# NikoBiele/RayTraceHeatTransfer.jl

Measured on AMD Instinct MI355X. Metric: Mrays/sec (exchange-factor trace), 101×101 grey κ=1 enclosure, 1/2/4/8 GPUs, higher is better.
Workload: dtype f64; 1 GPU; 101x101 grey kappa=1 sigma_s=0 unit-square enclosure (BASELINE configs[1]); 1e+08 rays per GPU, emitter rows sharded over 1 GPU(s); n_emitters=10605, rays_per_emitter=9429, parallelism=emitter-rows x1 (one process per GPU), devices_visible=1, seed=1

## Files before the change

raytraceheattransfer.jl_amd/csrc/rthx_api.cpp:

```cpp
#define RTHX_HOST_ONLY_TU 1
#include <hip/hip_runtime.h>

#include <algorithm>
#include <chrono>
#include <cmath>
#include <cstdio>
#include <cstdlib>
#include <cstring>
#include <mutex>
#include <string>
#include <thread>
#include <vector>

#include "../../include/rthx.h"
#include "rthx_grid.h"
#include "rthx_kernels.h"

#include "rthx_common.h"
#include "rthx_domain.h"

using rthx::DevBuf;
using rthx::HostBuf;
using rthx::fail;
using rthx::hip_fail;
// ... 438 lines not shown
      off = a16(off + 4 * cmap.size());
      G.off_cinfo = (int32_t)off;
      off = a16(off + sizeof(rthx::MCoarse) * nc);
      G.off_bsolid = (int32_t)off;
      off = a16(off + 4 * nc);
      G.off_beta = (int32_t)off;
      G.blob_bytes = (int32_t)off;
      off = a16(off + 8 * nc);
      if (ncx == 1) {
        G.off_lay = (int32_t)off;
        off = a16(off + sizeof(rthx::LayerRec) * (size_t)(ncy + 2));
      }
      G.inv_x = (double)nx / (xs[nx] - xs[0]);
      G.inv_y = (double)ny / (ys[ny] - ys[0]);
      G.inv_cx = (double)ncx / (cxs[ncx] - cxs[0]);
      G.inv_cy = (double)ncy / (cys[ncy] - cys[0]);
      if (off <= rthx::kMaxCoarseLdsBytes) {
        G.bytes = (int32_t)off;
        std::vector<uint4> blob((size_t)G.blob_bytes / 16);
        char* b = reinterpret_cast<char*>(blob.data());
        std::memset(b, 0, (size_t)G.blob_bytes);
        std::memcpy(b, xs.data(), 8 * xs.size());
        std::memcpy(b + G.off_ys, ys.data(), 8 * ys.size());
        std::memcpy(b + G.off_cxs, cxs.data(), 8 * cxs.size());
        std::memcpy(b + G.off_cys, cys.data(), 8 * cys.size());
        std::memcpy(b + G.off_cmap, cmap.data(), 4 * cmap.size());
        std::memcpy(b + G.off_cinfo, info.data(), sizeof(rthx::MCoarse) * nc);
        std::vector<uint32_t> bsolid(nc);
        std::vector<double> bbeta((size_t)s.n_bins * nc);
        for (size_t bx = 0; bx < nc; ++bx) {
          const int c = cmap[bx];
          bsolid[bx] = csolid[c];
          for (int bn = 0; bn < s.n_bins; ++bn) bbeta[(size_t)bn * nc + bx] = cbeta_all[(size_t)bn * nc + c];
        }
        std::memcpy(b + G.off_bsolid, bsolid.data(), 4 * nc);
        UP(blob.data(), blob.size(), D.ml_blob);
        UP(bbeta.data(), bbeta.size(), D.ml_bbeta);
        d->ml_mixed.assign((size_t)s.n_bins, 0);
        for (int bn = 0; bn < s.n_bins; ++bn)
          for (size_t bx = 0; bx < nc; ++bx) d->ml_mixed[bn] |= bbeta[(size_t)bn * nc + bx] < 0.0 ? 1 : 0;
        D.ml = G;
      }
    }
  }
  if (d->single_convex && d->axis_rect && !env_flag("RTHX_NO_LAT")) {
    std::vector<double> xs, ys;
    for (size_t f = 0; f < nf; ++f) {
      xs.push_back(fpoly[f].x[0]);
      xs.push_back(fpoly[f].x[1]);
      ys.push_back(fpoly[f].y[0]);
      ys.push_back(fpoly[f].y[2]);
    }
    std::sort(xs.begin(), xs.end());
    xs.erase(std::unique(xs.begin(), xs.end()), xs.end());
    std::sort(ys.begin(), ys.end());
    ys.erase(std::unique(ys.begin(), ys.end()), ys.end());
    const int64_t lnx = (int64_t)xs.size() - 1, lny = (int64_t)ys.size() - 1;
    bool ok = lnx >= 1 && lny >= 1 && lnx * lny == (int64_t)nf && lnx <= rthx::kLatMaxDim && lny <= rthx::kLatMaxDim;
    std::vector<int32_t> map(ok ? (size_t)(lnx * lny) : 0, -1);
    bool identity = ok;
    for (size_t f = 0; f < nf && ok; ++f) {
      const auto ix = std::lower_bound(xs.begin(), xs.end(), fpoly[f].x[0]) - xs.begin();
      const auto iy = std::lower_bound(ys.begin(), ys.end(), fpoly[f].y[0]) - ys.begin();
      ok = ix < lnx && iy < lny && xs[ix + 1] == fpoly[f].x[1] && ys[iy + 1] == fpoly[f].y[2] &&
           map[iy * lnx + ix] < 0;
      if (!ok) break;
      map[iy * lnx + ix] = (int32_t)f;
      identity = identity && (int64_t)f == iy * lnx + ix;
      const bool bnd[4] = {iy == 0, ix == lnx - 1, iy == lny - 1, ix == 0};
      for (int w = 0; w < 4 && ok; ++w) ok = bnd[w] || s.fine_surface[4 * f + w] < 0;
    }
    if (ok) {
      rthx::LatticeLayout L{};
      L.nx = (int32_t)lnx;
      L.ny = (int32_t)lny;
      L.identity = identity ? 1 : 0;
      auto a16 = [](size_t b) { return (b + 15) & ~(size_t)15; };
      size_t off = a16(8 * xs.size());
      L.off_ys = (int32_t)off;
      off = a16(off + 8 * ys.size());
      L.bytes = (int32_t)off;
      L.inv_x = (double)lnx / (xs[lnx] - xs[0]);
      L.inv_y = (double)lny / (ys[lny] - ys[0]);
      std::vector<uint4> blob(off / 16);
      char* b = reinterpret_cast<char*>(blob.data());
      std::memset(b, 0, off);
      std::memcpy(b, xs.data(), 8 * xs.size());
      std::memcpy(b + L.off_ys, ys.data(), 8 * ys.size());
      UP(blob.data(), blob.size(), D.lat_blob);
      if (!identity) UP(map.data(), map.size(), D.lat_map);
      D.lat = L;
    }
  }
#undef UP
  {
    int r3 = upload(d, &d->D, 1, &d->d_dom, "domain record");
    if (r3) return bail(r3);
  }
  *out = d;
  return RTHX_OK;
}

RTHX_EXPORT void rthx_domain_destroy(rthx_domain* dom) {
  if (!dom) return;
  (void)hipSetDevice(dom->device);
  (void)hipStreamSynchronize(dom->stream);
  delete dom;
}

RTHX_EXPORT int rthx_result_create(rthx_result** out) {
  if (!out) return fail(RTHX_EINVAL, "null out");
  *out = new (std::nothrow) rthx_result();
  return *out ? RTHX_OK : fail(RTHX_ENOMEM, "host allocation failed");
}

RTHX_EXPORT void rthx_result_destroy(rthx_result* res) { delete res; }

namespace rthx {

int finish_staged(rthx_result* res, const TallyParams& T, int merge, hipStream_t st, hipEvent_t ev_end,
                  int64_t totals[4]) {
  if (T.n_rows > 0) {
    if (merge == kMergeDense) HIP_TRY(launch_compact(T, st), "row_compact_kernel launch");
    if (merge == kMergeParts) HIP_TRY(launch_part_merge(T, st), "part_merge_kernel launch");
    HIP_TRY(launch_scan(T.row_nnz, T.row_tallied, T.n_rows, T.R, res->row_off.as<int64_t>(),
                        res->totals.as<int64_t>(), st),
            "row_scan_kernel launch");
  } else {
    HIP_TRY(hipMemsetAsync(res->row_off.p, 0, 8, st), "hipMemset");
  }
  HIP_TRY(hipMemcpyAsync(totals, res->totals.p, 32, hipMemcpyDeviceToHost, st), "hipMemcpy totals");
  HIP_TRY(hipStreamSynchronize(st), "row scan");
  const size_t nnz = (size_t)std::max<int64_t>(totals[0], 1);
  HIP_TRY(res->cols.reserve(nnz * 4), "hipMalloc cols");
  HIP_TRY(res->cnt.reserve(nnz * 4), "hipMalloc cnt");
  if (T.n_rows > 0)
    HIP_TRY(launch_pack(T.stage_cols, T.stage_cnt, T.row_cap, res->row_off.as<int64_t>(), T.n_rows,
                        res->cols.as<uint32_t>(), res->cnt.as<uint32_t>(), st),
            "csr_pack_kernel launch");
  HIP_TRY(hipEventRecord(ev_end, st), "hipEventRecord");
  HIP_TRY(hipStreamSynchronize(st), "CSR pack");
  return RTHX_OK;
}

}

namespace {

constexpr uint64_t kLookbackWaitTicks = 25'000'000;

uint64_t lookback_wait_ticks() {
  const char* e = rthx::knob("RTHX_LB_WAIT_US");
  if (e && *e) return (uint64_t)std::strtoull(e, nullptr, 10) * 100;
  return kLookbackWaitTicks;
}

using rthx::TracePlan;
static_assert(rthx::kTallyU16 == 1, "TracePlan::tally default");

constexpr int64_t kMaxHashCap = 16384;

int plan_trace(const rthx_domain* dom, const rthx_trace_args* a, TracePlan& p, int64_t slots = 0) {
  if (a->bin < 0 || a->bin >= dom->n_bins) return fail(RTHX_EINVAL, "bin out of range");
  if (a->rays_per_emitter < 0 || a->rays_per_emitter > 0xFFFFFFFFll)
    return fail(RTHX_ERANGE, "rays_per_emitter must be in [0, 2^32)");
  if (a->emitter_stride < 1 || a->emitter_begin < 0) return fail(RTHX_EINVAL, "bad emitter range");
// ... 836 lines not shown
```

raytraceheattransfer.jl_amd/csrc/rthx_device.h:

```cpp
#pragma once

#include <hip/hip_runtime.h>
#include <stdint.h>

#if defined(__HIP_DEVICE_COMPILE__) && !defined(RTHX_HOST_ONLY_TU)
#define RTHX_GLOBAL __attribute__((address_space(1)))
#else
#define RTHX_GLOBAL
#endif

#ifndef RTHX_PHILOX_OPAQUE_KEY
#define RTHX_PHILOX_OPAQUE_KEY 1
#endif

namespace rthx {

struct DevGrid {
  double ox, oy;
  double inv_x, inv_y;
  int32_t nx, ny;
  int32_t cell_base;
  int32_t reserved;
};

// ... 542 lines not shown
template <bool FAITHFUL>
__device__ __forceinline__ void iso_dir(uint32_t w_th, uint32_t w_ph, const double* cos_tab, double& dx, double& dy) {
  const double u = u32(w_th);
  double st, ct, cphi;
  if (FAITHFUL) {
    const double theta = acos(2.0 * u - 1.0);
    st = sin(theta);
    ct = cos(theta);
    cphi = cos(RTHX_TWO_PI * u32(w_ph));
  } else {
    ct = 2.0 * u - 1.0;
    st = 2.0 * sqrt_unit(__dmul_rn(u, 1.0 - u));
    cphi = cos_2pi_u32(w_ph, cos_tab);
  }
  dx = __dmul_rn(st, cphi);
  dy = ct;
}

template <bool FAITHFUL>
__device__ __forceinline__ void redirect_dir(bool wall, double tx, double ty, uint32_t w1, uint32_t w2,
                                             const double* cos_tab, double& dx, double& dy) {
  if (FAITHFUL) {
    if (wall)
      lambert_dir<true>(tx, ty, w1, w2, cos_tab, dx, dy);
    else
      iso_dir<true>(w1, w2, cos_tab, dx, dy);
    return;
  }
  const double u = u32(w1);
  const float ct_w = (float)sqrt_unit((double)(float)u);
  const double ct = wall ? (double)ct_w : 2.0 * u - 1.0;
  const double arg = wall ? 1.0 - (double)__fmul_rn(ct_w, ct_w) : 4.0 * __dmul_rn(u, 1.0 - u);
  const double st = sqrt_unit(arg);
  const double cpsi = cos_2pi_u32(wall ? f32_draw_word(w2) : w2, cos_tab);
  const double fx = wall ? tx : 1.0, fy = wall ? ty : 0.0;
  const double xl = __dmul_rn(st, cpsi);
  dx = __dmul_rn(fx, xl) + __dmul_rn(-fy, ct);
  dy = __dmul_rn(fy, xl) + __dmul_rn(fx, ct);
}

constexpr int kEmitAny = 0, kEmitVolRect = 2;
template <int EK> struct EmitKind { static constexpr int value = EK; };

template <bool FAITHFUL, int EK = kEmitAny>
__device__ __forceinline__ void emit_volume(const Emitter& e, double eta, const RayWords& rw, const double* cos_tab,
                                            double& px, double& py, double& dx, double& dy) {
  const double R1 = u32(rw.a[0]), R2 = u32(rw.a[1]);
  if (!FAITHFUL && (EK == kEmitVolRect || e.rect)) {
    px = __builtin_fma((double)rw.a[0], e.sx, e.v[0]);
    py = __builtin_fma((double)rw.a[1], e.sy, e.v[1]);
  } else {
    double s1 = FAITHFUL ? sqrt(R1) : sqrt_unit(R1);
    double wa = 1.0 - s1, wb = __dmul_rn(s1, 1.0 - R2), wc = __dmul_rn(s1, R2);
    double Ax = e.v[0], Ay = e.v[1], Bx = e.v[2], By = e.v[3], Cx = e.v[4], Cy = e.v[5];
    if (EK == kEmitVolRect || e.nv == 4) {
      double sel = u32(rw.sw);
      if (!(sel < e.tri_frac)) {
        Ax = e.v[4]; Ay = e.v[5]; Bx = e.v[6]; By = e.v[7]; Cx = e.v[0]; Cy = e.v[1];
      }
    }
    px = __dmul_rn(wa, Ax) + __dmul_rn(wb, Bx) + __dmul_rn(wc, Cx);
    py = __dmul_rn(wa, Ay) + __dmul_rn(wb, By) + __dmul_rn(wc, Cy);
  }
  px = px + __dmul_rn(e.mx - px, eta);
  py = py + __dmul_rn(e.my - py, eta);
  double st, ct, cphi;
  if (FAITHFUL) {
    double u4 = u32(rw.a[2]);
    double theta = acos(1.0 - 2.0 * u4);
    st = sin(theta);
    ct = cos(theta);
    cphi = cos(RTHX_TWO_PI * u32(rw.a[3]));
  } else {
    const double w4 = (double)rw.a[2];
    ct = __builtin_fma(w4, -0x1.0p-31, 1.0);
    const double om = __builtin_fma(w4, -0x1.0p-32, 1.0) * 0x1.0p-32;
    st = 2.0 * sqrt_unit(w4 * om);
    cphi = cos_2pi_u32(rw.a[3], cos_tab);
  }
  dx = __dmul_rn(st, cphi);
  dy = ct;
}

struct SingleCoarse {
  DevPoly poly;
  DevGrid grid;
  uint32_t solid;
  int32_t count;
};

constexpr int kRayContinue = -3;

template <bool UNIFORM, bool SINGLE, bool AXIS>
__device__ __forceinline__ int segment(const DevDomain& D, const TraceParams& P, const SingleCoarse& sc, int& c,
                                       double& px, double& py, double dx, double dy, double& S, double& acc) {
  const double eta = P.eta;
  int k, first, count;
  double u;
  uint32_t solid;
  if (SINGLE) {
    first = 0;
    count = sc.count;
    u = dist_to_cell<AXIS>(px, py, dx, dy, sc.poly, k);
    solid = sc.solid;
  } else {
    first = D.f_offset[c];
    count = D.f_offset[c + 1] - first;
    u = dist_to_cell<AXIS>(px, py, dx, dy, D.c_poly[c], k);
    solid = D.c_solid[c];
  }
  bool gas;
  double beta = 0.0, tau_b = 0.0;
  if (UNIFORM) {
    gas = S < u;
  } else {
    int f0 = SINGLE ? locate_fine(D, sc.grid, first, count, px, py) : locate_fine(D, D.f_grid[c], first, count, px, py);
    if (f0 < 0) return -1;
    beta = D.beta[(size_t)P.bin * D.n_fine + first + f0];
    tau_b = __dmul_rn(beta, u);
    gas = acc + tau_b >= S;
  }
  bool wall = !gas && ((solid >> k) & 1u);
  if (gas || wall) {
    double t = gas ? (UNIFORM ? S : (S - acc) / beta) - eta : u - eta;
    px = px + __dmul_rn(t, dx);
    py = py + __dmul_rn(t, dy);
    int f = SINGLE ? locate_fine(D, sc.grid, first, count, px, py) : locate_fine(D, D.f_grid[c], first, count, px, py);
    if (f < 0) return -1;
    int fg = first + f;
    if (gas) return D.n_surfaces + fg;
    int w;
    dist_to_cell<AXIS>(px, py, dx, dy, D.f_poly[fg], w);
    return D.f_surf[4 * fg + w];
  }
  if (SINGLE) return -1;
  double t = u + eta;
  px = px + __dmul_rn(t, dx);
  py = py + __dmul_rn(t, dy);
  if (UNIFORM) S -= u; else acc += tau_b;
  c = locate_coarse(D, px, py);
  return c < 0 ? -1 : kRayContinue;
}

#ifndef RTHX_LDS
#define RTHX_LDS __attribute__((address_space(3)))
#endif

__device__ __forceinline__ int lattice_index(const double RTHX_LDS* b, int n, double inv, double x) {
  int i;
  __asm__("v_cvt_i32_f64 %0, %1" : "=v"(i) : "v"(__dmul_rn(x - b[0], inv)));
  __asm__("v_med3_i32 %0, %1, 0, %2" : "=v"(i) : "v"(i), "s"(__builtin_amdgcn_readfirstlane(n - 1)));
  const double lo = b[i], hi = b[i + 1];
  if ((lo <= x) & (x < hi)) return i;
  while (i > 0 && x < b[i]) --i;
  while (i < n - 1 && !(x < b[i + 1])) ++i;
  return (b[i] <= x && x < b[i + 1]) ? i : -1;
}

static_assert(kLatMaxDim <= (1 << 12), "j nx + i must fit the 24-bit multiply and its 32-bit byte offsets");
__device__ __forceinline__ int lat_cell(int i, int j, int nx) {
  return (int)(__umul24((uint32_t)j, (uint32_t)nx) + (uint32_t)i);
}

template <class T>
__device__ __forceinline__ T ld_off32(const T RTHX_GLOBAL* base, uint32_t byte_off) {
  return *(const T RTHX_GLOBAL*)((const char RTHX_GLOBAL*)base + byte_off);
}

struct LatticeLds {
  const double RTHX_LDS* xs;
  const double RTHX_LDS* ys;
};

__device__ __forceinline__ LatticeLds lattice_lds_view(const char RTHX_LDS* base, const LatticeLayout& L) {
  LatticeLds v;
  v.xs = (const double RTHX_LDS*)base;
  v.ys = (const double RTHX_LDS*)(base + L.off_ys);
  return v;
}

template <bool UNIFORM, bool INSIDE = false, bool FOUR = false>
__device__ __forceinline__ int segment_lat(const DevDomain& D, const TraceParams& P, const SingleCoarse& sc,
                                           const LatticeLds& L, const LatticeLayout& G, double& px, double& py,
                                           double dx, double dy, double& S, double& acc) {
  const double eta = P.eta;
  int k;
  const double cx0 = sc.poly.x[0], cx1 = sc.poly.x[1], cy0 = sc.poly.y[0], cy1 = sc.poly.y[2];
  double u;
  if (!FOUR && (INSIDE || (cx0 <= px && px < cx1 && cy0 <= py && py < cy1)))
    u = dist_in_box(px, py, dx, dy, dx < 0.0 ? cx0 : cx1, dy < 0.0 ? cy0 : cy1, k);
  else
    u = dist_to_box(px, py, dx, dy, cx0, cx1, cy0, cy1, k);
  bool gas;
  double beta = 0.0, tau_b = 0.0;
  if (UNIFORM) {
    gas = S < u;
  } else {
    const int i0 = lattice_index(L.xs, G.nx, G.inv_x, px), j0 = lattice_index(L.ys, G.ny, G.inv_y, py);
    if (i0 < 0 || j0 < 0) return -1;
    const int f0 = G.identity ? lat_cell(i0, j0, G.nx) : D.lat_map[lat_cell(i0, j0, G.nx)];
    beta = D.beta[(size_t)P.bin * D.n_fine + f0];
    tau_b = __dmul_rn(beta, u);
    gas = acc + tau_b >= S;
  }
  const bool wall = !gas && ((sc.solid >> k) & 1u);
  if (!(gas || wall)) return -1;
  const double t = gas ? (UNIFORM ? S : (S - acc) / beta) - eta : u - eta;
  px = px + __dmul_rn(t, dx);
  py = py + __dmul_rn(t, dy);
  const int i = lattice_index(L.xs, G.nx, G.inv_x, px), j = lattice_index(L.ys, G.ny, G.inv_y, py);
  if (i < 0 || j < 0) return -1;
  const int cell = lat_cell(i, j, G.nx);
  if (gas) return D.n_surfaces + (G.identity ? cell : D.lat_map[cell]);
  const int w = box_hit_in(px, py, dx, dy, dx < 0.0 ? L.xs[i] : L.xs[i + 1], dy < 0.0 ? L.ys[j] : L.ys[j + 1]).wall;
  return ld_off32(D.f_surf, ((uint32_t)(G.identity ? cell : D.lat_map[cell]) << 4) + ((uint32_t)w << 2));
}

#ifndef RTHX_LDS
#define RTHX_LDS __attribute__((address_space(3)))
#endif

template <class T>
__device__ __forceinline__ T ld(const T RTHX_LDS* p) { return *(const T*)p; }
template <class T>
__device__ __forceinline__ T ld(const T RTHX_GLOBAL* p) { return *p; }

struct CoarseLds {
  const DevPoly RTHX_LDS* poly;
  const DevGrid RTHX_LDS* fgrid;
  const double RTHX_LDS* bbox;
  const int32_t RTHX_LDS* first;
  const uint32_t RTHX_LDS* solid;
  const DevCell RTHX_LDS* cells;
  const double RTHX_LDS* beta;
};

__device__ __forceinline__ CoarseLds coarse_lds_view(const char RTHX_LDS* base, const CoarseLayout& L) {
  CoarseLds v;
  v.poly = (const DevPoly RTHX_LDS*)base;
  v.fgrid = (const DevGrid RTHX_LDS*)(base + L.off_fgrid);
  v.bbox = (const double RTHX_LDS*)(base + L.off_bbox);
  v.first = (const int32_t RTHX_LDS*)(base + L.off_first);
  v.solid = (const uint32_t RTHX_LDS*)(base + L.off_solid);
  v.cells = (const DevCell RTHX_LDS*)(base + L.off_cells);
  v.beta = (const double RTHX_LDS*)(base + L.off_beta);
  return v;
}

constexpr int kRayEndGas = -4;
constexpr int kRayEndWall = -5;

template <bool UNIFORM, bool AXIS>
__device__ __forceinline__ int walk_cl(const DevDomain& D, const TraceParams& P, const CoarseLds& L, int& c,
                                       double& px, double& py, double dx, double dy, double& S, double& acc) {
  const double eta = P.eta;
  int k;
  const double u = dist_to_cell<AXIS>(px, py, dx, dy, L.poly[c], k);
  const uint32_t solid = L.solid[c];
  bool gas;
  double beta = 0.0, tau_b = 0.0;
  if (UNIFORM) {
    gas = S < u;
  } else {
    beta = L.beta[c];
    if (beta < 0.0) {
      const int first = L.first[c];
      const DevGrid fg = ld(L.fgrid + c);
      const int f0 = locate_fine(D, fg, first, L.first[c + 1] - first, px, py);
      if (f0 < 0) return -1;
      beta = D.beta[(size_t)P.bin * D.n_fine + first + f0];
    }
    tau_b = __dmul_rn(beta, u);
    gas = acc + tau_b >= S;
  }
  const bool wall = !gas && ((solid >> k) & 1u);
  if (gas || wall) {
    const double t = gas ? (UNIFORM ? S : (S - acc) / beta) - eta : u - eta;
    px = px + __dmul_rn(t, dx);
    py = py + __dmul_rn(t, dy);
    return gas ? kRayEndGas : kRayEndWall;
  }
  const double t = u + eta;
  px = px + __dmul_rn(t, dx);
  py = py + __dmul_rn(t, dy);
  if (UNIFORM) S -= u; else acc += tau_b;
  c = locate(D.c_grid, D, L.cells, L.poly, L.bbox, 0, D.n_coarse, px, py);
  return c < 0 ? -1 : kRayContinue;
}

template <bool AXIS>
__device__ __forceinline__ int end_cl(const DevDomain& D, const CoarseLds& L, int c, double px, double py, double dx,
                                      double dy, bool gas) {
  const int first = L.first[c];
  const DevGrid fg = ld(L.fgrid + c);
  const int f = locate_fine(D, fg, first, L.first[c + 1] - first, px, py);
  if (f < 0) return -1;
  const int fg_idx = first + f;
  if (gas) return D.n_surfaces + fg_idx;
// ... 267 lines not shown
        if (beta < 0.0) {
          const MCoarse m = ld(L.cinfo + L.cmap[cj]);
          int i, j;
          const int f0 = ml_fine(L, G, m, px, py, i, j);
          lost = f0 < 0;
          beta = lost ? 0.0 : D.beta[(size_t)P.bin * D.n_fine + f0];
        }
      }
      accn = acc + __dmul_rn(beta, u);
      gas = accn >= S;
    }
    const bool wall = !gas & ((rec.solid & ybit) != 0u);
    if ((it >= kMaxWalkSteps) | !fast | lost | gas | wall) {
      status = it >= kMaxWalkSteps ? -1 : !fast ? kRaySlowSeg : lost ? -1 : gas ? kRayEndGas : kRayEndWall;
      break;
    }
    const double t = u + eta;
    px = px + __dmul_rn(t, r.dx);
    py = py + __dmul_rn(t, r.dy);
    if (UNIFORM) S -= u; else acc = accn;
    cj += sy;
    ++it;
    if ((uint32_t)__popcll(__ballot(1)) <= stop) break;
  }
  u_end = u;
  B.ci = 0;
  B.cj = cj;
  B.b = cj;
  return status;
}

__device__ __forceinline__ bool relocate_layers(const MLatLds& L, const MLatLayout& G, MBox& B, double px,
                                                double py) {
  const int li = lattice_index(L.cxs, 1, G.inv_cx, px), lj = lattice_index(L.cys, G.ncy, G.inv_cy, py);
  if ((li < 0) | (lj < 0)) return false;
  B.ci = 0;
  B.cj = lj;
  B.b = lj;
  return true;
}

template <bool UNIFORM>
__device__ __forceinline__ void end_move_ml(const DevDomain& D, const TraceParams& P, const MLatLds& L,
                                            const MLatLayout& G, const MBox& B, double& px, double& py,
                                            const MRay& r, double S, double acc, double u_end, bool gas) {
  double t = u_end;
  if (gas) {
    if (UNIFORM) {
      t = S;
    } else {
      double beta = L.beta[B.b];
      if (P.mixed && beta < 0.0) {
        const MCoarse m = ld(L.cinfo + L.cmap[B.b]);
        int i, j;
        beta = D.beta[(size_t)P.bin * D.n_fine + ml_fine(L, G, m, px, py, i, j)];
      }
      t = (S - acc) / beta;
    }
  }
  t = t - P.eta;
  px = px + __dmul_rn(t, r.dx);
  py = py + __dmul_rn(t, r.dy);
}

__device__ __forceinline__ int end_ml(const DevDomain& D, const MLatLds& L, const MLatLayout& G, const MBox& B,
                                      double px, double py, double dx, double dy, bool gas) {
  const MCoarse m = ld(L.cinfo + L.cmap[B.b]);
  int i, j;
  const int fg = ml_fine(L, G, m, px, py, i, j);
  if (fg < 0) return -1;
  if (gas) return D.n_surfaces + fg;
  const int w = box_hit_in(px, py, dx, dy, dx < 0.0 ? L.xs[i] : L.xs[i + 1], dy < 0.0 ? L.ys[j] : L.ys[j + 1]).wall;
  return D.f_surf[4 * fg + w];
}

template <bool UNIFORM, bool FAITHFUL>
__device__ __forceinline__ double free_path(const TraceParams& P, const double* tabs, double u) {
  if (UNIFORM)
    return FAITHFUL ? (P.beta_uniform > 0 ? -log(u) / P.beta_uniform : __builtin_inf())
                    : neg_log_tab(u, tabs + kLogTableOffset) * tabs[kTabInvBeta];
  return FAITHFUL ? -log(u) : neg_log_tab(u, tabs + kLogTableOffset);
}

template <bool UNIFORM, bool FAITHFUL>
__device__ __forceinline__ double free_path_u32(const TraceParams& P, const double* tabs, uint32_t w) {
  if (FAITHFUL) return free_path<UNIFORM, true>(P, tabs, u32(w));
  const double l = neg_log_u32(w, tabs + kLogTableOffset);
  if (UNIFORM) return l * tabs[kTabInvBeta];
  return l;
}

template <int EK = kEmitAny>
__device__ __forceinline__ bool emitter_surface(const Emitter& e) { return EK == kEmitAny ? e.surface : false; }

template <int EK = kEmitAny>
__device__ __forceinline__ RayWords ray_words(const TraceParams& P, const Emitter& e, uint32_t g, uint32_t r,
                                              bool have_pw, uint32_t pw, bool faithful) {
  RayWords rw;
  philox_words(r, g, 0u, (uint32_t)P.bin, P.key0, P.key1, rw.a);
  rw.pw = 0u;
  rw.sw = 0u;
  if (!emitter_surface<EK>(e)) {
    if (have_pw) {
      rw.pw = pw;
    } else {
      uint32_t b[4];
      philox_words(r >> 2, g, 1u, (uint32_t)P.bin, P.key0, P.key1, b);
      const uint32_t j = r & 3u;
      rw.pw = j == 0 ? b[0] : j == 1 ? b[1] : j == 2 ? b[2] : b[3];
    }
    if (EK == kEmitVolRect ? faithful : (e.need_sel || (faithful && e.nv == 4))) {
      uint32_t c[4];
      philox_words(r, g, 2u, (uint32_t)P.bin, P.key0, P.key1, c);
      rw.sw = c[0];
    }
  }
  return rw;
}

template <bool UNIFORM, bool FAITHFUL, int EK = kEmitAny>
__device__ __forceinline__ void start_ray_w(const TraceParams& P, const Emitter& e, const double* tabs,
                                            const RayWords& rw, double& px, double& py, double& dx, double& dy,
                                            double& S) {
  const bool surface = emitter_surface<EK>(e);
  if (surface)
    emit_surface<FAITHFUL>(e, P.eta, rw, tabs, px, py, dx, dy);
  else
    emit_volume<FAITHFUL, EK>(e, P.eta, rw, tabs, px, py, dx, dy);
  uint32_t w_surf = rw.a[3], w_vol = rw.pw;
  __asm__ volatile("" : "+v"(w_surf), "+v"(w_vol));
  S = free_path_u32<UNIFORM, FAITHFUL>(P, tabs, surface ? w_surf : w_vol);
}

template <bool UNIFORM, bool FAITHFUL>
__device__ __forceinline__ void start_ray(const TraceParams& P, const Emitter& e, const double* tabs, uint32_t g,
                                          uint32_t r, double& px, double& py, double& dx, double& dy, double& S) {
  const RayWords rw = ray_words(P, e, g, r, false, 0u, FAITHFUL);
  start_ray_w<UNIFORM, FAITHFUL>(P, e, tabs, rw, px, py, dx, dy, S);
}

template <bool UNIFORM, bool FAITHFUL, bool SINGLE, bool AXIS, bool LAT = false, int EK = kEmitAny>
__device__ __forceinline__ int trace_one_w(const DevDomain& D, const TraceParams& P, const Emitter& e,
                                           const SingleCoarse& sc, const double* tabs, const RayWords& rw,
                                           double& ox, double& oy, double& px, double& py,
                                           const char RTHX_LDS* lat_base = nullptr) {
  double dx, dy, S, acc = 0.0;
  start_ray_w<UNIFORM, FAITHFUL, EK>(P, e, tabs, rw, px, py, dx, dy, S);
  ox = px;
  oy = py;
  if (LAT)
    return segment_lat<UNIFORM, EK == kEmitVolRect>(D, P, sc, lattice_lds_view(lat_base, D.lat), D.lat, px, py, dx,
                                                     dy, S, acc);
  int c = e.coarse;
  for (int it = 0; it < (SINGLE ? 1 : 10000); ++it) {
    const int a = segment<UNIFORM, SINGLE, AXIS>(D, P, sc, c, px, py, dx, dy, S, acc);
    if (a != kRayContinue) return a;
  }
  return -1;
}

}
```

raytraceheattransfer.jl_amd/csrc/rthx_kernels.hip:

```cpp
#include <hip/hip_runtime.h>
#include <stdint.h>

#include <algorithm>
#include <map>
#include <mutex>

#include "rthx_device.h"
#include "rthx_kernels.h"
#include "rthx_partition.h"
#include "rthx_wave.h"

namespace rthx {

#ifndef RTHX_TRACE_WAVES_PER_EU
#define RTHX_TRACE_WAVES_PER_EU 5
#endif
#ifndef RTHX_LAT_WAVES_PER_EU
#define RTHX_LAT_WAVES_PER_EU 8
#endif
#ifndef RTHX_MULTI_WAVES_PER_EU
#define RTHX_MULTI_WAVES_PER_EU 4
#endif
#define RTHX_ML_VIEW mlat_lds_view(lds_opaque(cl_base), D.ml)
#define RTHX_ML_G D.ml
// ... 295 lines not shown
  extern __shared__ uint32_t hist[];
  const DevDomain& D = *Dp;
  __shared__ uint32_t wave_sum[kMaxTraceThreads / 64];
  __shared__ uint32_t s_tallied;
  __shared__ uint32_t s_next;
  __shared__ Emitter s_emit;
  __shared__ SingleCoarse s_single;
#if RTHX_GTAB
  const double* const g_tab = (const double*)((const double RTHX_GLOBAL*)D.tables + (size_t)P.bin * kLdsTableDoubles);
#define RTHX_TAB_PTR g_tab
#else
  __shared__ double s_tab[kLdsTableDoubles];
#define RTHX_TAB_PTR ((const double*)lds_opaque(&s_tab[0]))
#endif

  constexpr bool CLDS = CL != 0;
  constexpr bool MLAT = CL == 2 && !SINGLE;
  const int tid = threadIdx.x;
  const uint32_t bid = blockIdx.x;
  constexpr bool tail = SPLIT;
  const uint32_t parts = SPLIT ? (uint32_t)T.split : 1u;
  const uint32_t trow = SPLIT ? bid / parts : bid;
  const uint32_t tpart = SPLIT ? bid - trow * parts : 0u;
  const int64_t slot = trow;
  const int64_t part = tpart;
  const uint32_t chunk = SPLIT ? (uint32_t)((P.R + parts - 1) / parts) : (uint32_t)P.R;
  constexpr bool kBase = RBASE || !SINGLE;
  const int64_t ray_base = kBase ? P.ray_base : 0;
  const int64_t p_begin = SPLIT ? (int64_t)(tpart * chunk) : 0;
  const int64_t r_begin = kBase ? ray_base + (p_begin < P.R ? p_begin : P.R) : p_begin;
  const int64_t r_end = kBase ? ray_base + (SPLIT ? (p_begin + chunk < P.R ? p_begin + chunk : P.R) : P.R)
                              : (SPLIT ? (r_begin + chunk < P.R ? r_begin + chunk : P.R) : P.R);
  const int64_t g = P.g_begin + slot * P.g_stride;
  constexpr bool PACK16 = TALLY == kTallyU16, HASH = TALLY == kTallyHash;
  const int64_t n_words = HASH ? 2 * (int64_t)T.hash_cap + T.bm_words : PACK16 ? (T.n_emitters + 1) / 2 : T.n_emitters;

  const int nthr = (int)blockDim.x;
  const int64_t z_words = SPLIT && !HASH ? (n_words + 3) & ~int64_t(3) : n_words;
  for (int64_t w = tid; w < z_words; w += nthr) hist[w] = 0u;
  char RTHX_LDS* cl_base = (char RTHX_LDS*)hist + T.cl_offset;
  if (CLDS && SINGLE) {
    uint4* dst = (uint4*)cl_base;
    for (int i = tid; i < D.lat.bytes / 16; i += nthr) dst[i] = D.lat_blob[i];
  } else if (MLAT) {
    uint4* dst = (uint4*)cl_base;
    for (int i = tid; i < D.ml.blob_bytes / 16; i += nthr) dst[i] = D.ml_blob[i];
    double RTHX_LDS* cb = (double RTHX_LDS*)(cl_base + D.ml.off_beta);
    for (int i = tid; i < D.n_coarse; i += nthr) cb[i] = D.ml_bbeta[(size_t)P.bin * D.n_coarse + i];
    if (D.ml.off_lay > 0) {
      LayerRec* lay = (LayerRec*)(cl_base + D.ml.off_lay);
      const char RTHX_GLOBAL* blob = (const char RTHX_GLOBAL*)D.ml_blob;
      const double RTHX_GLOBAL* cys = (const double RTHX_GLOBAL*)(blob + D.ml.off_cys);
      const uint32_t RTHX_GLOBAL* bs = (const uint32_t RTHX_GLOBAL*)(blob + D.ml.off_bsolid);
      for (int i = tid; i < D.ml.ncy + 2; i += nthr) {
        const bool layer = i >= 1 && i <= D.ml.ncy;
        LayerRec r;
        r.y0 = layer ? cys[i - 1] : __builtin_nan("");
        r.y1 = layer ? cys[i] : __builtin_nan("");
        r.beta = layer ? D.ml_bbeta[(size_t)P.bin * D.n_coarse + i - 1] : 0.0;
        r.solid = layer ? bs[i - 1] : 0u;
        r.pad = 0u;
        lay[i] = r;
      }
    }
  } else if (CLDS) {
    uint4* dst = (uint4*)cl_base;
    for (int i = tid; i < D.cl.blob_bytes / 16; i += nthr) dst[i] = D.c_blob[i];
    double RTHX_LDS* cb = (double RTHX_LDS*)(cl_base + D.cl.off_beta);
    for (int i = tid; i < D.n_coarse; i += nthr) cb[i] = D.c_beta[(size_t)P.bin * D.n_coarse + i];
  }
#if !RTHX_GTAB
  if (!FAITHFUL)
    for (int i = tid; i < kLdsTableDoubles; i += nthr) s_tab[i] = i < kTableDoubles ? D.tables[i] : P.inv_beta_uniform;
#endif
  if (tid == 0) {
    s_tallied = 0u;
    s_next = (uint32_t)r_begin;
    s_emit = load_emitter(D, g);
    if (SINGLE) {
      s_single.poly = D.c_poly[0];
      s_single.grid = D.f_grid[0];
      s_single.solid = D.c_solid[0];
      s_single.count = D.f_offset[1];
    }
  }
  int rec_slot = -1;
  if (REC)
    for (int i = 0; i < rec.n; ++i)
      if (rec.ids[i] == g) { rec_slot = i; break; }
  __syncthreads();

  uint32_t tallied = 0;
  auto tally = [&](int a) {
    if (a >= 0) {
      if (HASH)
        hash_tally(hist, hist + T.hash_cap, (uint32_t)T.hash_cap - 1u, (uint32_t)T.hash_shift, (uint32_t)a);
      else if (PACK16)
        atomicAdd(&hist[a >> 1], 1u << ((uint32_t)(a & 1) << 4));
      else
        atomicAdd(&hist[a], 1u);
      ++tallied;
    }
  };
  auto record = [&](uint32_t r, int a, double ox, double oy, double px, double py) {
    if (REC && rec_slot >= 0) {
      size_t k = (size_t)rec_slot * (size_t)P.R + (size_t)(r - (uint32_t)ray_base);
      rec.ok[k] = a >= 0 ? 1 : 0;
      rec.orig[2 * k] = ox; rec.orig[2 * k + 1] = oy;
      rec.end[2 * k] = px; rec.end[2 * k + 1] = py;
    }
  };
  if (SINGLE) {
    auto one_ray = [&](uint32_t r, bool have_pw, uint32_t pw, auto ek) {
      constexpr int EK = decltype(ek)::value;
      double ox, oy, px, py;
      const SingleCoarse RTHX_LDS* sc = lds_opaque(&s_single);
      const double* tab = RTHX_TAB_PTR;
      const Emitter RTHX_LDS* em = lds_opaque(&s_emit);
      const Emitter& e = *(const Emitter*)em;
      const RayWords rw = ray_words<EK>(P, e, (uint32_t)g, r, have_pw, pw, FAITHFUL);
      int a = trace_one_w<UNIFORM, FAITHFUL, SINGLE, AXIS, CLDS && AXIS, EK>(
          D, P, e, *(const SingleCoarse*)sc, (const double*)tab, rw, ox, oy, px, py, lds_opaque(cl_base));
      tally(a);
      record(r, a, ox, oy, px, py);
    };
    const uint32_t rb = (uint32_t)r_begin;
    const uint32_t re = (uint32_t)r_end > rb ? (uint32_t)r_end : rb;
    const uint32_t q0 = rb >> 2, q1 = (re + 3u) >> 2;
    const uint32_t nt = (uint32_t)__builtin_amdgcn_readfirstlane(nthr);
    const bool volume = __builtin_amdgcn_readfirstlane((int)lds_opaque(&s_emit)->surface) == 0;
    const bool vrect = volume && __builtin_amdgcn_readfirstlane((int)lds_opaque(&s_emit)->rect) != 0;
    const uint32_t n_rd = (uint32_t)__builtin_amdgcn_readfirstlane((int)((q1 - q0 + nt - 1u) / nt));
    auto rounds = [&](auto ek) {
    uint32_t q = q0 + (uint32_t)tid;
    uint32_t q_lo = q0;
    for (uint32_t rd = 0; rd < n_rd; ++rd, q += nt, q_lo += nt) {
      if (q < q1) {
        uint32_t b[4] = {0u, 0u, 0u, 0u};
        if (volume) philox_words(q, (uint32_t)g, 1u, (uint32_t)P.bin, P.key0, P.key1, b);
        const bool edge = (rd == 0u && (rb & 3u) != 0u) || (q_lo + nt >= q1 && (re & 3u) != 0u);
#if RTHX_ROUND_UNROLL
#pragma unroll
#else
#pragma nounroll
#endif
        for (uint32_t k = 0; k < 4u; ++k) {
          uint32_t r = 4u * q + k;
          const uint32_t pw = k == 0u ? b[0] : k == 1u ? b[1] : k == 2u ? b[2] : b[3];
          bool in = true;
          if (edge) {
            __asm__ volatile("" : "+v"(r));
            in = r >= rb && r < re;
          }
          if (in) one_ray(r, true, pw, ek);
        }
      }
    }
    };
    if constexpr (!FAITHFUL) {
      if (vrect)
        rounds(EmitKind<kEmitVolRect>{});
      else
        rounds(EmitKind<kEmitAny>{});
    } else {
      (void)vrect;
      rounds(EmitKind<kEmitAny>{});
    }
  } else if constexpr (MLAT) {
    constexpr uint32_t kRefillQ = RTHX_REFILL_Q;
    const uint32_t lane = lane_id();
    const uint64_t lt_mask = lane == 0 ? 0ull : (~0ull >> (64 - lane));
    double RTHX_LDS* q = (double RTHX_LDS*)(cl_base + D.ml.bytes) + (tid >> 6) * (64 * kRaySlotDoubles);
    __shared__ MBox s_box0;
#ifdef RTHX_SEGSTAT
    __shared__ unsigned long long s_segs;
    if (tid == 0) s_segs = 0ull;
#endif
    if (tid == 0) ml_enter(mlat_lds_view(cl_base, D.ml), D.ml, s_emit.coarse, s_box0);
    __syncthreads();
    uint32_t q_head = 0, q_cnt = 0;
    bool exhausted = false;
    const bool layered = D.ml.ncx == 1;
    double px = 0.0, py = 0.0, S = 0.0, acc = 0.0, u_end = 0.0;
    MRay ry{};
    int it = 0;
    MBox box{};
    int state = -1;
    while (true) {
      if (state == kRaySlowSeg) {
        int cj = box.cj;
        state = P.mixed ? layer_segment<UNIFORM, true>(D, P, RTHX_ML_VIEW, RTHX_ML_G, cj, px, py, ry, S, acc, it, u_end)
                        : layer_segment<UNIFORM, false>(D, P, RTHX_ML_VIEW, RTHX_ML_G, cj, px, py, ry, S, acc, it, u_end);
        box.ci = 0;
        box.cj = cj;
        box.b = cj;
      }
      if (state == kRayEndGas || state == kRayEndWall) {
        const bool gas = state == kRayEndGas;
        end_move_ml<UNIFORM>(D, P, RTHX_ML_VIEW, RTHX_ML_G, box, px, py, ry, S, acc, u_end, gas);
        tally(end_ml(D, RTHX_ML_VIEW, RTHX_ML_G, box, px, py, ry.dx, ry.dy, gas));
      }
      if (state == kRayRelocate)
        state = relocate_layers(RTHX_ML_VIEW, RTHX_ML_G, box, px, py) ? kRayContinue : -1;
      bool live = state == kRayContinue;
      const uint64_t idle = __ballot(!live);
      const uint32_t n_idle = (uint32_t)__popcll(idle);
      if (!exhausted && q_cnt < n_idle) {
        const uint32_t want = 64u - q_cnt;
        uint32_t base = 0;
        if (lane == 0) base = atomicAdd(&s_next, want);
        base = __shfl(base, 0);
        const uint32_t rr = base + lane;
        const bool valid = lane < want && rr < (uint32_t)r_end;
        if (valid) {
          const double* tab = RTHX_TAB_PTR;
          const Emitter RTHX_LDS* em = lds_opaque(&s_emit);
          const Emitter& e = *(const Emitter*)em;
          double v[kRaySlotDoubles];
          start_ray<UNIFORM, FAITHFUL>(P, e, (const double*)tab, (uint32_t)g, rr, v[0], v[1], v[2], v[3], v[4]);
          v[5] = 1.0 / fabs(v[2]);
          v[6] = 1.0 / fabs(v[3]);
          double RTHX_LDS* d = q + ((q_head + q_cnt + lane) & 63u);
#pragma unroll
          for (int f = 0; f < kRaySlotDoubles; ++f) d[64 * f] = v[f];
        }
        const uint32_t n_new = (uint32_t)__popcll(__ballot(valid));
        if (n_new < want) exhausted = true;
        q_cnt += n_new;
      }
      if (q_cnt > 0) {
        const uint32_t rank = (uint32_t)__popcll(idle & lt_mask);
        if (!live && rank < q_cnt) {
          const double RTHX_LDS* sl = q + ((q_head + rank) & 63u);
          px = sl[0];
          py = sl[64];
          ry.dx = sl[128];
          ry.dy = sl[192];
          S = sl[256];
          ry.rax = sl[320];
          ry.ray = sl[384];
          acc = 0.0;
          it = 0;
          box = s_box0;
          live = true;
        }
        const uint32_t taken = q_cnt < n_idle ? q_cnt : n_idle;
        q_head = (q_head + taken) & 63u;
        q_cnt -= taken;
      }
      state = live ? kRayContinue : -1;
// ... 640 lines not shown
```

Measured before the change: 146,500 Mrays/s.

## Add branch-light lattice fast path for single-coarse uniform rays with rare fixup

Adds a specialised per-ray path for single-coarse, axis-aligned, uniform-medium traces. It computes the exit cell with a clamped index guess and one bounds check. Rays whose guess misses, or that leave the domain, fall back to a lattice-walk fixup. Grid parameters and inv_beta are packed into LDS padding inside SingleCoarse, and tallies use a branch-free atomic (masked/zero-valued for out-of-range rays) with a bulk tally count. The aim is to cut divergent lattice searches and per-ray bookkeeping, at the cost of more code paths, subtle tally-accounting logic and a new env knob that rescales the guess.

```diff
diff --git a/raytraceheattransfer.jl_amd/csrc/rthx_api.cpp b/raytraceheattransfer.jl_amd/csrc/rthx_api.cpp
--- a/raytraceheattransfer.jl_amd/csrc/rthx_api.cpp
+++ b/raytraceheattransfer.jl_amd/csrc/rthx_api.cpp
@@ -544,6 +544,13 @@
       L.bytes = (int32_t)off;
       L.inv_x = (double)lnx / (xs[lnx] - xs[0]);
       L.inv_y = (double)lny / (ys[lny] - ys[0]);
+      if (const char* gs = rthx::knob("RTHX_LAT_GUESS_SCALE")) {
+        const double sc = std::strtod(gs, nullptr);
+        if (std::isfinite(sc) && sc > 0.0) {
+          L.inv_x *= sc;
+          L.inv_y *= sc;
+        }
+      }
       std::vector<uint4> blob(off / 16);
       char* b = reinterpret_cast<char*>(blob.data());
       std::memset(b, 0, off);
diff --git a/raytraceheattransfer.jl_amd/csrc/rthx_device.h b/raytraceheattransfer.jl_amd/csrc/rthx_device.h
--- a/raytraceheattransfer.jl_amd/csrc/rthx_device.h
+++ b/raytraceheattransfer.jl_amd/csrc/rthx_device.h
@@ -648,12 +648,29 @@
   dy = ct;
 }
 
+struct LatGrid {
+  double x0, y0;
+  double inv_x, inv_y;
+  int32_t nxm1, nym1;
+  int32_t nx;
+  int32_t off_ys;
+};
+static_assert(sizeof(LatGrid) == sizeof(DevGrid), "LatGrid overlays SingleCoarse::grid");
+
 struct SingleCoarse {
   DevPoly poly;
-  DevGrid grid;
+  union {
+    DevGrid grid;
+    LatGrid lat;
+  };
   uint32_t solid;
-  int32_t count;
-};
+  union {
+    int32_t count;
+    int32_t n_surfaces;
+  };
+  double inv_beta;
+};
+static_assert(sizeof(SingleCoarse) == 192, "SingleCoarse fills the padding it had: the kernels' static LDS is unchanged");
 
 constexpr int kRayContinue = -3;
 
@@ -780,6 +797,114 @@
   if (gas) return D.n_surfaces + (G.identity ? cell : D.lat_map[cell]);
   const int w = box_hit_in(px, py, dx, dy, dx < 0.0 ? L.xs[i] : L.xs[i + 1], dy < 0.0 ? L.ys[j] : L.ys[j + 1]).wall;
   return ld_off32(D.f_surf, ((uint32_t)(G.identity ? cell : D.lat_map[cell]) << 4) + ((uint32_t)w << 2));
+}
+
+struct LatRay {
+  double px, py;
+  double dx, dy;
+  double S;
+  bool gas;
+  bool lost;
+  bool cold;
+};
+
+__device__ __forceinline__ int lattice_walk(const double RTHX_LDS* b, int nm1, int i, double x) {
+#pragma unroll 1
+  while (true) {
+    const bool dn = i > 0 && x < b[i];
+    const bool up = !dn && i < nm1 && !(x < b[i + 1]);
+    if (!(dn | up)) break;
+    i += dn ? -1 : 1;
+  }
+  return (b[i] <= x && x < b[i + 1]) ? i : -1;
+}
+
+__device__ __forceinline__ int lattice_guess(double x, double x0, double inv, int nm1) {
+  int i;
+  __asm__("v_cvt_i32_f64 %0, %1" : "=v"(i) : "v"(__dmul_rn(x - x0, inv)));
+  __asm__("v_med3_i32 %0, %1, 0, %2" : "=v"(i) : "v"(i), "v"(nm1));
+  return i;
+}
+
+#ifndef RTHX_LAT_SURF_MASKED
+#define RTHX_LAT_SURF_MASKED 1
+#endif
+
+template <bool INSIDE>
+__device__ __forceinline__ int lat_ray_fast(const DevDomain& D, double eta, const SingleCoarse& sc,
+                                            const char RTHX_LDS* lat_base, bool identity, bool cold0, LatRay& r) {
+  const double ox = r.px, oy = r.py, dx = r.dx, dy = r.dy, S = r.S;
+  const double cx0 = sc.poly.x[0], cx1 = sc.poly.x[1], cy0 = sc.poly.y[0], cy1 = sc.poly.y[2];
+  const bool xdn = dx < 0.0, ydn = dy < 0.0;
+  const bool y_first = ydn | xdn;
+  double u;
+  int k;
+  if (INSIDE) {
+    const double xb = xdn ? cx0 : cx1, yb = ydn ? cy0 : cy1;
+    const double sx = xb - ox, sy = yb - oy;
+    const double mx = __dmul_rn(fabs(sx), fabs(dx)), my = __dmul_rn(fabs(sy), fabs(dy));
+    const bool vx = (fabs(dx) >= 1e-10) & (mx > 0.0);
+    const bool vy = (fabs(dy) >= 1e-10) & (my > 0.0);
+    const double cx = __dmul_rn(fabs(sx), fabs(dy)), cy = __dmul_rn(fabs(sy), fabs(dx));
+    const bool xw = vx & (!vy | (y_first & (cx < cy)) | (!y_first & !(cy < cx)));
+    const bool any = vx | vy;
+    const double q = div_pos(fabs(xw ? sx : sy), fabs(xw ? dx : dy));
+    u = any ? q : __builtin_inf();
+    k = any ? (xw ? (xdn ? 3 : 1) : (ydn ? 0 : 2)) : 0;
+  } else {
+    if (cx0 <= ox && ox < cx1 && cy0 <= oy && oy < cy1)
+      u = dist_in_box(ox, oy, dx, dy, xdn ? cx0 : cx1, ydn ? cy0 : cy1, k);
+    else
+      u = dist_to_box(ox, oy, dx, dy, cx0, cx1, cy0, cy1, k);
+  }
+  const bool gas = S < u;
+  const bool wall = !gas & (((sc.solid >> k) & 1u) != 0u);
+  const bool lost = !(gas | wall);
+  const double t = (gas ? S : u) - eta;
+  const double px = ox + __dmul_rn(t, dx);
+  const double py = oy + __dmul_rn(t, dy);
+  r.px = px;
+  r.py = py;
+  r.gas = gas;
+  r.lost = lost;
+  const LatGrid& G = sc.lat;
+  const double RTHX_LDS* xs = (const double RTHX_LDS*)lat_base;
+  const double RTHX_LDS* ys = (const double RTHX_LDS*)(lat_base + G.off_ys);
+  const int i = lattice_guess(px, G.x0, G.inv_x, G.nxm1);
+  const int j = lattice_guess(py, G.y0, G.inv_y, G.nym1);
+  const double xlo = xs[i], xhi = xs[i + 1], ylo = ys[j], yhi = ys[j + 1];
+  const bool hit = (xlo <= px) & (px < xhi) & (ylo <= py) & (py < yhi);
+  int f = lat_cell(i, j, G.nx);
+  if (!identity) f = D.lat_map[f];
+  const double sx = (xdn ? xlo : xhi) - px, sy = (ydn ? ylo : yhi) - py;
+  const double mx = __dmul_rn(fabs(sx), fabs(dx)), my = __dmul_rn(fabs(sy), fabs(dy));
+  const bool vx = (fabs(dx) >= 1e-10) & (mx > 0.0);
+  const bool vy = (fabs(dy) >= 1e-10) & (my > 0.0);
+  const double cx = __dmul_rn(fabs(sx), fabs(dy)), cy = __dmul_rn(fabs(sy), fabs(dx));
+  const bool xw = vx & (!vy | (y_first & (cx < cy)) | (!y_first & !(cy < cx)));
+  const int wl = xw ? (xdn ? 3 : 1) : (ydn ? 0 : 2);
+  int surf = -1;
+  if (!RTHX_LAT_SURF_MASKED || wall) surf = ld_off32(D.f_surf, ((uint32_t)f << 4) + ((uint32_t)wl << 2));
+  const int a = gas ? sc.n_surfaces + f : surf;
+  r.cold = cold0 | lost | !hit | (wall & !(vx | vy)) | (a < 0);
+  return a;
+}
+
+__device__ __forceinline__ int lat_ray_fixup(const DevDomain& D, const SingleCoarse& sc,
+                                             const char RTHX_LDS* lat_base, bool identity, const LatRay& r) {
+  if (r.lost) return -1;
+  const double px = r.px, py = r.py, dx = r.dx, dy = r.dy;
+  const LatGrid& G = sc.lat;
+  const double RTHX_LDS* xs = (const double RTHX_LDS*)lat_base;
+  const double RTHX_LDS* ys = (const double RTHX_LDS*)(lat_base + G.off_ys);
+  const int i = lattice_walk(xs, G.nxm1, lattice_guess(px, G.x0, G.inv_x, G.nxm1), px);
+  const int j = lattice_walk(ys, G.nym1, lattice_guess(py, G.y0, G.inv_y, G.nym1), py);
+  if (i < 0 || j < 0) return -1;
+  int f = lat_cell(i, j, G.nx);
+  if (!identity) f = D.lat_map[f];
+  if (r.gas) return sc.n_surfaces + f;
+  const int w = box_hit_in(px, py, dx, dy, dx < 0.0 ? xs[i] : xs[i + 1], dy < 0.0 ? ys[j] : ys[j + 1]).wall;
+  return ld_off32(D.f_surf, ((uint32_t)f << 4) + ((uint32_t)w << 2));
 }
 
 #ifndef RTHX_LDS
@@ -1213,11 +1338,12 @@
   return FAITHFUL ? -log(u) : neg_log_tab(u, tabs + kLogTableOffset);
 }
 
-template <bool UNIFORM, bool FAITHFUL>
-__device__ __forceinline__ double free_path_u32(const TraceParams& P, const double* tabs, uint32_t w) {
+template <bool UNIFORM, bool FAITHFUL, bool LATRAY = false>
+__device__ __forceinline__ double free_path_u32(const TraceParams& P, const double* tabs, uint32_t w,
+                                                const SingleCoarse* sc = nullptr) {
   if (FAITHFUL) return free_path<UNIFORM, true>(P, tabs, u32(w));
   const double l = neg_log_u32(w, tabs + kLogTableOffset);
-  if (UNIFORM) return l * tabs[kTabInvBeta];
+  if (UNIFORM) return l * (LATRAY ? sc->inv_beta : tabs[kTabInvBeta]);
   return l;
 }
 
@@ -1249,10 +1375,10 @@
   return rw;
 }
 
-template <bool UNIFORM, bool FAITHFUL, int EK = kEmitAny>
+template <bool UNIFORM, bool FAITHFUL, int EK = kEmitAny, bool LATRAY = false>
 __device__ __forceinline__ void start_ray_w(const TraceParams& P, const Emitter& e, const double* tabs,
                                             const RayWords& rw, double& px, double& py, double& dx, double& dy,
-                                            double& S) {
+                                            double& S, const SingleCoarse* sc = nullptr) {
   const bool surface = emitter_surface<EK>(e);
   if (surface)
     emit_surface<FAITHFUL>(e, P.eta, rw, tabs, px, py, dx, dy);
@@ -1260,7 +1386,7 @@
     emit_volume<FAITHFUL, EK>(e, P.eta, rw, tabs, px, py, dx, dy);
   uint32_t w_surf = rw.a[3], w_vol = rw.pw;
   __asm__ volatile("" : "+v"(w_surf), "+v"(w_vol));
-  S = free_path_u32<UNIFORM, FAITHFUL>(P, tabs, surface ? w_surf : w_vol);
+  S = free_path_u32<UNIFORM, FAITHFUL, LATRAY>(P, tabs, surface ? w_surf : w_vol, sc);
 }
 
 template <bool UNIFORM, bool FAITHFUL>
diff --git a/raytraceheattransfer.jl_amd/csrc/rthx_kernels.hip b/raytraceheattransfer.jl_amd/csrc/rthx_kernels.hip
--- a/raytraceheattransfer.jl_amd/csrc/rthx_kernels.hip
+++ b/raytraceheattransfer.jl_amd/csrc/rthx_kernels.hip
@@ -401,6 +401,21 @@
       s_single.grid = D.f_grid[0];
       s_single.solid = D.c_solid[0];
       s_single.count = D.f_offset[1];
+      if (CLDS && AXIS) {
+        const char RTHX_GLOBAL* blob = (const char RTHX_GLOBAL*)D.lat_blob;
+        LatGrid lg;
+        lg.x0 = *(const double RTHX_GLOBAL*)blob;
+        lg.y0 = *(const double RTHX_GLOBAL*)(blob + D.lat.off_ys);
+        lg.inv_x = D.lat.inv_x;
+        lg.inv_y = D.lat.inv_y;
+        lg.nxm1 = D.lat.nx - 1;
+        lg.nym1 = D.lat.ny - 1;
+        lg.nx = D.lat.nx;
+        lg.off_ys = D.lat.off_ys;
+        s_single.lat = lg;
+        s_single.n_surfaces = D.n_surfaces;
+        s_single.inv_beta = P.inv_beta_uniform;
+      }
     }
   }
   int rec_slot = -1;
@@ -442,6 +457,42 @@
           D, P, e, *(const SingleCoarse*)sc, (const double*)tab, rw, ox, oy, px, py, lds_opaque(cl_base));
       tally(a);
       record(r, a, ox, oy, px, py);
+    };
+    constexpr bool LATRAY = CLDS && AXIS && UNIFORM && !RBASE;
+    const bool lat_identity = LATRAY && __builtin_amdgcn_readfirstlane(D.lat.identity) != 0;
+    auto one_ray_lat = [&](uint32_t r, uint32_t pw, bool cold0, auto ek) {
+      constexpr int EK = decltype(ek)::value;
+      const SingleCoarse RTHX_LDS* scl = lds_opaque(&s_single);
+      const SingleCoarse& sc = *(const SingleCoarse*)scl;
+      const double* tab = RTHX_TAB_PTR;
+      const Emitter RTHX_LDS* em = lds_opaque(&s_emit);
+      const Emitter& e = *(const Emitter*)em;
+      const RayWords rw = ray_words<EK>(P, e, (uint32_t)g, r, true, pw, FAITHFUL);
+      LatRay ry;
+      start_ray_w<UNIFORM, FAITHFUL, EK, true>(P, e, (const double*)tab, rw, ry.px, ry.py, ry.dx, ry.dy, ry.S, &sc);
+      const char RTHX_LDS* lat = lds_opaque(cl_base);
+      int a = lat_ray_fast<EK == kEmitVolRect>(D, P.eta, sc, lat, lat_identity, cold0, ry);
+      auto fixup = [&]() {
+        int a2 = -1;
+        if (!cold0) {
+          a2 = lat_ray_fixup(D, sc, lat, lat_identity, ry);
+          if (a2 < 0) atomicSub(&s_tallied, 1u);
+        }
+        return a2;
+      };
+      if constexpr (HASH) {
+        if (ry.cold) a = fixup();
+        if (a >= 0) hash_tally(hist, hist + T.hash_cap, (uint32_t)T.hash_cap - 1u, (uint32_t)T.hash_shift, (uint32_t)a);
+      } else {
+        uint32_t word = PACK16 ? (uint32_t)a >> 1 : (uint32_t)a;
+        uint32_t val = PACK16 ? 1u << ((uint32_t)(a & 1) << 4) : 1u;
+        if (ry.cold) {
+          const int a2 = fixup();
+          word = a2 < 0 ? 0u : PACK16 ? (uint32_t)a2 >> 1 : (uint32_t)a2;
+          val = a2 < 0 ? 0u : PACK16 ? 1u << ((uint32_t)(a2 & 1) << 4) : 1u;
+        }
+        atomicAdd(&hist[word], val);
+      }
     };
     const uint32_t rb = (uint32_t)r_begin;
     const uint32_t re = (uint32_t)r_end > rb ? (uint32_t)r_end : rb;
@@ -458,6 +509,27 @@
         uint32_t b[4] = {0u, 0u, 0u, 0u};
         if (volume) philox_words(q, (uint32_t)g, 1u, (uint32_t)P.bin, P.key0, P.key1, b);
         const bool edge = (rd == 0u && (rb & 3u) != 0u) || (q_lo + nt >= q1 && (re & 3u) != 0u);
+        if constexpr (LATRAY) {
+          bool out[4] = {false, false, false, false};
+          if (edge) {
+#pragma unroll
+            for (uint32_t k = 0; k < 4u; ++k) {
+              uint32_t r = 4u * q + k;
+              __asm__ volatile("" : "+v"(r));
+              out[k] = !(r >= rb && r < re);
+            }
+          }
+#if RTHX_ROUND_UNROLL
+#pragma unroll
+#else
+#pragma nounroll
+#endif
+          for (uint32_t k = 0; k < 4u; ++k) {
+            const uint32_t pw = k == 0u ? b[0] : k == 1u ? b[1] : k == 2u ? b[2] : b[3];
+            const bool o = k == 0u ? out[0] : k == 1u ? out[1] : k == 2u ? out[2] : out[3];
+            one_ray_lat(4u * q + k, pw, o, ek);
+          }
+        } else {
 #if RTHX_ROUND_UNROLL
 #pragma unroll
 #else
@@ -473,6 +545,7 @@
           }
           if (in) one_ray(r, true, pw, ek);
         }
+        }
       }
     }
     };
@@ -485,6 +558,7 @@
       (void)vrect;
       rounds(EmitKind<kEmitAny>{});
     }
+    if constexpr (LATRAY) tallied = tid == 0 ? re - rb : 0u;
   } else if constexpr (MLAT) {
     constexpr uint32_t kRefillQ = RTHX_REFILL_Q;
     const uint32_t lane = lane_id();
```

Result: faster. 153,400 Mrays/s (median of 6 runs) (+4.7%).
